# openjamoses/TOSEM-2021-Replication

Measured on NVIDIA H100. Metric: source MB/s scanned (tokenise + line-hash + classify + aggregate), higher is better.
Workload: dtype u8

## Files before the change

### tosem-2021-replication_b200/csrc/tsm_api.cu

```cuda
#include <algorithm>
#include <cstdio>
#include <cstdlib>
#include <cstring>
#include <new>
#include <vector>

#include "tsm_device.cuh"

#include "tsm_scan_kernels.cuh"
#include "tsm_scan_walk.cuh"
#include "tsm_reduce_kernels.cuh"
#include "tsm_diff_kernels.cuh"
#include "tsm_stmt_kernels.cuh"
#include "tsm_lines_kernels.cuh"

using namespace tsm;

static const char* const kNames[TSM_K] = TSM_CAT_NAMES_INIT;

struct ScratchPool {
  struct Slot { void* p; size_t cap; bool used; };
  std::vector<Slot> slots;
  void* take(size_t bytes) {
    int best = -1;
// ... 379 lines not shown
        }
      }
      p.slab = c->d_slab + s; p.f_begin = f0; p.f_end = f1;
      p.unit_base = (uint32_t)((host ? (int64_t)host->off[f0] : 0) / CH + f0);
      k_plan<<<(f1 - f0 + 255) / 256, 256, 0, st>>>(p);
      CU(cudaGetLastError());
      if (s == 0 && n_slabs == 1) CU(cudaEventRecord(ev[1], st));
      if (flags & TSM_SCAN_REV_B) k_scan_t<true><<<c->sms * SCAN2_CTAS_PER_SM, SCAN2_WARPS * 32, SCAN2_SMEM_B, st>>>(p);
      else k_scan_t<false><<<c->sms * SCAN2_CTAS_PER_SM, SCAN2_WARPS * 32, SCAN2_SMEM, st>>>(p);
      CU(cudaGetLastError());
      if (s + 1 < n_slabs) {
        p.cls_last = 0;
        if (flags & TSM_SCAN_REV_B) k_classify_t<true><<<c->cls_grid, 256, hist, st>>>(p);
        else k_classify_t<false><<<c->cls_grid, 256, hist, st>>>(p);
        CU(cudaGetLastError());
        p.cls_last = 1;
      }
    }
    if (n_slabs > 1) CU(cudaEventRecord(ev[1], st));
    CU(cudaEventRecord(ev[2], st));
    if (flags & TSM_SCAN_REV_B) k_classify_t<true><<<c->cls_grid, 256, hist, st>>>(p);
    else k_classify_t<false><<<c->cls_grid, 256, hist, st>>>(p);
    CU(cudaGetLastError());
    CU(cudaEventRecord(ev[3], st));
    CU(cudaEventRecord(ev[4], st));
    c->ev_used[es] = (n_slabs == 1);
    c->ev_last = es;
    c->launches = 3 * n_slabs;
    CU(cudaGetLastError());
  }
  c->last_flags = flags;
  c->scanned = true;
  return TSM_OK;
}

extern "C" int tsm_scan_resident(tsm_ctx* c, uint32_t flags, void* stream) {
  if (!c) return TSM_E_ARG;
  flags &= TSM_SCAN_ASSERT_EVENTS | TSM_SCAN_HEADER_EVENTS | TSM_SCAN_REV_B;
  if (!c->resident) return TSM_E_STATE;
  CU(cudaSetDevice(c->device));
  return launch_scan(c, flags, (cudaStream_t)stream, nullptr);
}

extern "C" int tsm_device_counts(tsm_ctx* c, void** dptr, int64_t* n_int64) {
  if (!c || !dptr || !n_int64) return TSM_E_ARG;
  if (!c->scanned) return TSM_E_STATE;
  *dptr = c->d_counts;
  *n_int64 = (int64_t)(c->n_groups + 1) * TSM_K + 4;
  return TSM_OK;
}

extern "C" int tsm_last_launch_count(tsm_ctx* c) { return c ? c->launches : 0; }

extern "C" int tsm_last_kernel_ms(tsm_ctx* c, float* ms4) {
  if (!c || !ms4) return TSM_E_ARG;
  if (!c->scanned || c->n_files == 0 || c->ev_last < 0) return TSM_E_STATE;
  CU(cudaSetDevice(c->device));
  cudaEvent_t* ev = c->ev[c->ev_last];
  CU(cudaEventSynchronize(ev[4]));
  for (int i = 0; i < 4; ++i) CU(cudaEventElapsedTime(&ms4[i], ev[i], ev[i + 1]));
  return TSM_OK;
}

extern "C" int tsm_kernel_ms_stats(tsm_ctx* c, double* sum_ms4, int64_t* n_scans, int reset) {
  if (!c) return TSM_E_ARG;
  CU(cudaSetDevice(c->device));
  for (int i = 0; i < tsm_ctx::kRing; ++i) fold_events(c, i);
  if (sum_ms4) for (int k = 0; k < 4; ++k) sum_ms4[k] = c->ms_sum[k];
  if (n_scans) *n_scans = c->ms_n;
  if (reset) { for (double& v : c->ms_sum) v = 0; c->ms_n = 0; }
  return TSM_OK;
}

extern "C" int tsm_download(tsm_ctx* c, tsm_result* r, void* stream) {
  if (!c || !r) return TSM_E_ARG;
  if (!c->scanned) return TSM_E_STATE;
  CU(cudaSetDevice(c->device));
  cudaStream_t st = (cudaStream_t)stream;
  const int n = c->n_files, G = c->n_groups;
  unsigned long long* h_tot = reinterpret_cast<unsigned long long*>(c->h_ctrl + 1);
  CU(cudaMemcpyAsync(c->h_ctrl, c->d_ctrl, sizeof(Ctrl), cudaMemcpyDeviceToHost, st));
  CU(cudaMemcpyAsync(h_tot, c->d_counts + (size_t)(G + 1) * TSM_K, 4 * sizeof(unsigned long long), cudaMemcpyDeviceToHost, st));
  if (r->stats && n) CU(cudaMemcpyAsync(r->stats, c->d_stats, sizeof(tsm_file_stat) * (size_t)n, cudaMemcpyDeviceToHost, st));
  if (r->group_counts) CU(cudaMemcpyAsync(r->group_counts, c->d_counts, sizeof(int64_t) * (size_t)G * TSM_K, cudaMemcpyDeviceToHost, st));
  if (r->global_counts) CU(cudaMemcpyAsync(r->global_counts, c->d_counts + (size_t)G * TSM_K, sizeof(int64_t) * TSM_K, cudaMemcpyDeviceToHost, st));
  CU(cudaStreamSynchronize(st));
  for (int i = 0; i < 4; ++i) r->totals[i] = (int64_t)h_tot[i];
  r->n_aev = 0; r->n_hev = 0;
  if (c->h_ctrl->overflow) return TSM_E_CAPACITY;
  if ((c->last_flags & TSM_SCAN_ASSERT_EVENTS) && r->aev) {
    const int64_t m = c->h_ctrl->n_aev;
    if (m > r->aev_cap) { r->n_aev = m; return TSM_E_CAPACITY; }
    CU(cudaMemcpyAsync(r->aev, c->d_aev, sizeof(tsm_assert_event) * (size_t)m, cudaMemcpyDeviceToHost, st));
    CU(cudaStreamSynchronize(st));
    std::sort(r->aev, r->aev + m, [](const tsm_assert_event& a, const tsm_assert_event& b) {
      return a.file != b.file ? a.file < b.file : a.line_off < b.line_off; });
    r->n_aev = m;
  } else if (c->last_flags & TSM_SCAN_ASSERT_EVENTS) r->n_aev = c->h_ctrl->n_aev;
  if ((c->last_flags & TSM_SCAN_HEADER_EVENTS) && r->hev) {
    const int64_t m = c->h_ctrl->n_hev;
    if (m > r->hev_cap) { r->n_hev = m; return TSM_E_CAPACITY; }
    CU(cudaMemcpyAsync(r->hev, c->d_hev, sizeof(tsm_header_event) * (size_t)m, cudaMemcpyDeviceToHost, st));
    CU(cudaStreamSynchronize(st));
    std::sort(r->hev, r->hev + m, [](const tsm_header_event& a, const tsm_header_event& b) {
      return a.file != b.file ? a.file < b.file : a.line_off < b.line_off; });
    r->n_hev = m;
// ... 523 lines not shown
```

### tosem-2021-replication_b200/csrc/tsm_scan_kernels.cuh

```cuda
#pragma once
#include <type_traits>
#include "tsm_device.cuh"

namespace tsm {

__constant__ uint32_t c_lut[256];
__constant__ uint32_t c_lut_b[256];
__constant__ uint32_t c_elut[256];
__device__ uint8_t c_cat_slot[TSM_CAT_SLOTS];
__device__ uint16_t c_cat_off[TSM_CAT_NAMED + 1];
__device__ char c_cat_blob[TSM_CAT_BLOB_LEN + 1];

__global__ void k_plan(ScanParams p) {
  const int f = p.f_begin + blockIdx.x * blockDim.x + threadIdx.x;
  const int lane = threadIdx.x & 31;
  if (blockIdx.x == 0 && threadIdx.x == 0) p.ctrl->cls_done = p.ctrl->n_cand;
  uint32_t nu = 0;
  if (f < p.f_end) {
    nu = ((uint32_t)p.len[f] + CH - 1) / CH;
    if (nu != 1) p.stats[f] = tsm_file_stat{0, 0, 0, 0, 0};
  }
  uint32_t incl = nu;
#pragma unroll
  for (int d = 1; d < 32; d <<= 1) {
// ... 112 lines not shown
template <typename LoadByte>
__device__ __forceinline__ uint32_t line_finish_h(uint32_t s, uint32_t e, unsigned long long h0, uint32_t nib, int ext,
                                                  LoadByte lb, Accum& ac) {
  uint32_t len = e - s;
  unsigned long long h = 0;
  if (len) {
    h = h0;
    if (lb(e - 1) == 0x0D) {
      --len;
      const unsigned long long cr = rotl61(0x0Dull, (8u * len) % 61u);
      h = h >= cr ? h - cr : h + M61 - cr;
    }
  }
  ac.lines++;
  ac.digest += mix_hash(h, len);
  if (ext == 0) return 0;
  uint32_t fl = (nib & 1u) ? LF_CAND : 0;
  bool hdr;
  if (ext == TSM_EXT_PY) {
    hdr = (nib & 2u) != 0;
    if (!hdr && (nib & 4u)) hdr = starts_with(lb, s, e, "class", 5, true);
  } else {
    hdr = (nib & 6u) == 6u;
  }
  if (hdr) { fl |= LF_HDR; if (starts_with(lb, s, e, "TEST_F", 6, false)) fl |= LF_FIX; }
  ac.asserts += fl & LF_CAND;
  ac.hdrs += (fl >> 1) & 1u;
  ac.fixes += (fl >> 2) & 1u;
  return fl;
}

template <typename LoadByte>
__device__ __forceinline__ uint32_t line_finish(uint32_t s, uint32_t e, uint32_t A, unsigned long long B, int ext,
                                                LoadByte lb, Accum& ac) {
  unsigned long long h0 = 0;
  if (e != s) {
    const uint32_t lead = s & 7u, m = ((e - 1) >> 3) - (s >> 3) + 1;
    h0 = rotl61(canon61(B), (3u * (m - 1) + 61u * 8u - 8u * lead) % 61u);
  }
  return line_finish_h(s, e, h0, ext ? flag_nibble_ext(A, ext) : 0u, ext, lb, ac);
}

__device__ __forceinline__ uint32_t warp_reserve(uint32_t* counter, uint32_t n, int lane) {
  uint32_t base = 0;
  if (lane == 0 && n) base = atomicAdd(counter, n);
  return __shfl_sync(0xffffffffu, base, 0);
}

__device__ __forceinline__ const uint32_t* scan_lut() {
  extern __shared__ __align__(128) uint8_t smem[];
  return reinterpret_cast<const uint32_t*>(smem);
}

__device__ __noinline__ uint32_t long_line(const ScanParams& p, const uint32_t* lut, uint32_t first, uint32_t f,
                                           uint32_t fo, uint32_t size, int ext, uint32_t s, Accum& ac, uint32_t* fl_out = nullptr) {
  const uint8_t* g = p.arena + fo;
  const GmemByte lb{g};
  uint32_t e = s;
  while (e < size && lb(e) != '\n') ++e;
  LineState L;
  line_init(L, s, e);
  while (L.pos < L.e) {
    const unsigned long long w = __ldg(reinterpret_cast<const unsigned long long*>(g + L.pos));
    line_block(L, w, lut, first);
  }
  const uint32_t fl = line_finish(s, e, L.A, L.B, ext, lb, ac);
  if ((fl & LF_CAND) && p.cand_cap) {
    const uint32_t slot = atomicAdd(&p.ctrl->n_cand, 1u);
    if (slot < p.cand_cap) p.cand[slot] = ((unsigned long long)f << 32) | s;
    else p.ctrl->overflow = 1;
  }
  if ((fl & LF_HDR) && (p.flags & TSM_SCAN_HEADER_EVENTS)) {
    const uint32_t slot = atomicAdd(&p.ctrl->n_hev, 1u);
    if (slot < p.hev_cap) p.hev[slot] = tsm_header_event{f, s, e - s, (fl >> 2) & 1u};
    else p.ctrl->overflow = 1;
  }
  if (fl_out) *fl_out = fl;
  return e;
}

__device__ __forceinline__ void issue_load(const ScanParams& p, uint8_t* buf, uint64_t* bar, uint32_t fo,
                                           uint32_t size, uint32_t cb) {
  const uint32_t lb = cb ? cb - PRE : 0u;
  const uint32_t le = min(cb + CH + EXT, size);
  const uint32_t bytes = (le - lb + 15u) & ~15u;
  mbar_expect_tx(bar, bytes);
  bulk_load(buf + PRE - (cb - lb), p.arena + (size_t)fo + lb, bytes, bar);
}

struct Unit { uint32_t u, f, cb, fo, size; int ext; };

__device__ __forceinline__ Unit claim_unit(const ScanParams& p, uint32_t n_units, int lane) {
  Unit x{0, 0, 0, 0, 0, 0};
  if (lane == 0) x.u = atomicAdd(&p.slab->work, 1u);
  x.u = __shfl_sync(0xffffffffu, x.u, 0);
  if (x.u < n_units) {
    x.f = p.unit_file[p.unit_base + x.u];
    x.cb = p.unit_begin[p.unit_base + x.u];
    x.fo = (uint32_t)p.off[x.f];
    x.size = (uint32_t)p.len[x.f];
    x.ext = p.ext[x.f];
  }
  return x;
}

constexpr uint32_t CC_W = 1, CC_IDENT = 2, CC_STOP = 4;
constexpr uint32_t CLS_CAT_OFF_N = (TSM_CAT_NAMED + 2) & ~1u;
constexpr uint32_t CLS_CAT_WORDS = ((TSM_CAT_SLOTS + 2 * CLS_CAT_OFF_N + TSM_CAT_BLOB_LEN + 15) / 16) * 4;
constexpr uint32_t CLS_SMEM_BASE = 4 * (512 + CLS_CAT_WORDS + 4 * 1024 + 4);
constexpr uint32_t E_FIRST = (1u << 0) | (1u << 5) | (1u << 9) | (1u << 17) | (1u << 21) | (1u << 23) | (1u << 25) |
                             (1u << 27) | (1u << 29) | (1u << 30);

struct FileBytes {
  const unsigned long long* base; uint32_t cur_blk; unsigned long long w;
  uint32_t blk0; unsigned long long w0, w1, w2, w3;
  __device__ __forceinline__ FileBytes(const uint8_t* b, uint32_t first_byte)
      : base(reinterpret_cast<const unsigned long long*>(b)), cur_blk(0xFFFFFFFFu), w(0), blk0(first_byte >> 3) {
    w0 = __ldg(base + blk0); w1 = __ldg(base + blk0 + 1); w2 = __ldg(base + blk0 + 2); w3 = __ldg(base + blk0 + 3);
  }
  __device__ __forceinline__ unsigned long long word(uint32_t blk) const {
    const uint32_t d = blk - blk0;
    if (d < 4u) return d < 2u ? (d == 0u ? w0 : w1) : (d == 2u ? w2 : w3);
    return __ldg(base + blk);
  }
  __device__ __forceinline__ uint32_t get(uint32_t i) {
    const uint32_t blk = i >> 3;
    if (blk != cur_blk) { w = word(blk); cur_blk = blk; }
    return (uint32_t)(w >> (8u * (i & 7u))) & 0xFFu;
  }
  __device__ __forceinline__ unsigned long long get8(uint32_t i) const {
    const uint32_t blk = i >> 3, sh = 8u * (i & 7u);
// ... 271 lines not shown
```

### tosem-2021-replication_b200/csrc/tsm_scan_walk.cuh

```cuda
#pragma once
#include "tsm_scan_kernels.cuh"

namespace tsm {

#ifndef TSM_SCAN2_WARPS
#define TSM_SCAN2_WARPS 11
#endif
#ifndef TSM_SCAN2_CTAS
#define TSM_SCAN2_CTAS 2
#endif
#ifndef TSM_RW2_SHIFT
#define TSM_RW2_SHIFT 2
#endif
#ifndef TSM_WALK_UNROLL
#define TSM_WALK_UNROLL 1
#endif
constexpr int SCAN2_WARPS = TSM_SCAN2_WARPS, SCAN2_CTAS_PER_SM = TSM_SCAN2_CTAS, WALK_UNROLL = TSM_WALK_UNROLL;

constexpr uint32_t NWORD = BUF / 8;
constexpr uint32_t O2_ARUN = BUF;
constexpr uint32_t SLOT_TAIL = NWORD;
constexpr uint32_t RW2_SHIFT = TSM_RW2_SHIFT, RW2_PER_STRIPE = 16u >> RW2_SHIFT;
constexpr uint32_t O2_RW = O2_ARUN + ((NWORD + 1) * 4 + 7) / 8 * 8;
constexpr uint32_t O2_WENT = O2_RW + 32 * RW2_PER_STRIPE * 8;
constexpr uint32_t WENT_CAP = NWORD + 8;
constexpr uint32_t LCAP = 512;
constexpr uint32_t O2_LTAB = O2_WENT + WENT_CAP * 2;
constexpr uint32_t O2_BASE = O2_LTAB + (LCAP + 8) * 2;
constexpr uint32_t Q2_CAP = 64;
constexpr uint32_t O2_Q = O2_BASE + 34 * 8;
constexpr uint32_t O2_CTL = O2_Q + Q2_CAP * 2;
constexpr uint32_t WARP_SMEM2 = ((O2_CTL + 16 + 127) / 128) * 128;
constexpr uint32_t O2_T0A = LUT_BYTES;
constexpr uint32_t CTA_BYTES2 = LUT_BYTES + 512;
constexpr uint32_t SCAN2_SMEM = CTA_BYTES2 + SCAN2_WARPS * WARP_SMEM2;
constexpr uint32_t O2_LUTB = SCAN2_SMEM;
constexpr uint32_t SCAN2_SMEM_B = SCAN2_SMEM + 1024;
static_assert(O2_RW % 8 == 0 && O2_WENT % 8 == 0 && O2_LTAB % 2 == 0 && O2_BASE % 8 == 0 && O2_Q % 4 == 0 && O2_CTL % 8 == 0, "alignment");
static_assert(SCAN2_CTAS_PER_SM * (SCAN2_SMEM_B + 1024) <= 233472, "shared memory per SM (228 KB, 1 KB reserved per CTA)");
constexpr uint32_t LR_POS = 0x1FFFu, LR_FIRST = 0x2000u, LR_MIXED = 0x4000u, LR_VIRT = 0x8000u;

constexpr uint32_t B2_FIRST = (1u << 0) | (1u << 6) | (1u << 15), B2_FIN = (1u << 5) | (1u << 14) | (1u << 18);
constexpr uint32_t REVB_BIT = 1u;

#ifndef TSM_PIPE_BALANCE
#define TSM_PIPE_BALANCE 1
#endif
template <bool REVB>
__device__ __forceinline__ void lut_at(uint32_t idx, uint32_t four, uint32_t& v, uint32_t& v2) {
#if TSM_PIPE_BALANCE
  uint32_t addr;
  asm("mad.lo.u32 %0, %1, %2, %3;" : "=r"(addr) : "r"(idx), "r"(four), "r"(smem_u32(scan_lut())));
  asm("ld.shared.u32 %0, [%1];" : "=r"(v) : "r"(addr));
  if (REVB) asm("ld.shared.u32 %0, [%1+%2];" : "=r"(v2) : "r"(addr), "n"(O2_LUTB));
#else
  (void)four;
  v = scan_lut()[idx];
  if (REVB) v2 = scan_lut()[O2_LUTB / 4 + idx];
#endif
}
__device__ __forceinline__ uint32_t opaque_four() { return scan_lut()[256 + 12]; }

struct Auto { uint32_t D, D2; };

template <bool REVB>
__device__ __forceinline__ uint32_t step1(Auto& a, uint32_t byte, uint32_t four) {
  uint32_t m, m2 = 0;
  lut_at<REVB>(byte, four, m, m2);
  a.D = ((a.D + a.D) | B_FIRST) & m;
  if (!REVB) return a.D;
  a.D2 = ((a.D2 + a.D2) | B2_FIRST) & m2;
  return (a.D & ~REVB_BIT) | ((a.D2 & B2_FIN) ? REVB_BIT : 0u);
}

template <bool REVB>
__device__ __forceinline__ void step8b(unsigned long long w, Auto& a, uint32_t& A, uint32_t four) {
  const uint32_t lo = (uint32_t)w, hi = (uint32_t)(w >> 32);
  uint32_t A2 = 0;
#pragma unroll
  for (int k = 0; k < 8; ++k) {
    uint32_t m, m2 = 0;
    lut_at<REVB>(__byte_perm(k < 4 ? lo : hi, 0, 0x4440 + (k & 3)), four, m, m2);
    a.D = ((a.D + a.D) | B_FIRST) & m;
    A |= a.D;
    if (REVB) { a.D2 = ((a.D2 + a.D2) | B2_FIRST) & m2; A2 |= a.D2; }
  }
  if (REVB) A = (A & ~REVB_BIT) | ((A2 & B2_FIN) ? REVB_BIT : 0u);
}

__device__ __forceinline__ uint32_t nl8_of(unsigned long long w) {
  return nl_word((uint32_t)w) | (nl_word((uint32_t)(w >> 32)) << 4);
}
__device__ __forceinline__ unsigned long long low_mask(uint32_t b) {
  return b >= 8u ? ~0ull : ((1ull << (8u * b)) - 1ull);
}
__device__ __forceinline__ unsigned long long ror3_61(unsigned long long r) { return (r >> 3) + ((r & 7ull) << 58); }

struct WalkOut { uint32_t nlw, tail; };

template <bool REVB>
__device__ __noinline__ WalkOut walk2(uint8_t* wb, uint32_t fin, int lane) {
  const uint32_t pos0 = (uint32_t)lane * STRIPE;
  const uint8_t* sp = wb + pos0;
  uint32_t* ar = reinterpret_cast<uint32_t*>(wb + O2_ARUN) + (uint32_t)lane * 17u;
  unsigned long long* rw = reinterpret_cast<unsigned long long*>(wb + O2_RW) + (uint32_t)lane * RW2_PER_STRIPE;
  const uint32_t four = opaque_four();
  Auto au{0u, 0u};
  if (lane) {
    uint32_t A = 0;
    step8b<REVB>(*reinterpret_cast<const unsigned long long*>(sp - 8), au, A, four);
  }
  unsigned long long R = 0;
  uint32_t run = 0, nlr = 0;
#pragma unroll 1
  for (uint32_t g = 0; g < 5; ++g) {
#pragma unroll WALK_UNROLL
    for (uint32_t k = 0; k < 4; ++k) {
      if (g == 4 && k) break;
      const unsigned long long w = *reinterpret_cast<const unsigned long long*>(sp + 32u * g + 8u * k);
      uint32_t A = 0;
      step8b<REVB>(w, au, A, four);
      R = ror3_61(R) + fold61(w);
      if (((k + 1u) & ((1u << RW2_SHIFT) - 1u)) == 0u && g < 4u) rw[(4u * g + k) >> RW2_SHIFT] = R;
      ar[4u * g + k] = run;
      nlr = __funnelshift_l(A, nlr, 1);
      const bool nl = (int32_t)A < 0;
      if (nl && (A & fin)) {
        const uint32_t slot = atomicAdd(reinterpret_cast<uint32_t*>(wb + O2_CTL), 1u);
        if (slot < Q2_CAP) reinterpret_cast<uint16_t*>(wb + O2_Q)[slot] = (uint16_t)((uint32_t)lane * 17u + 4u * g + k);
      }
      run = nl ? 0u : (run | A);
    }
  }
  unsigned long long incl = rotl61(canon61(R), (3u * (17u * (uint32_t)lane + 16u)) % 61u);
#pragma unroll
  for (int d = 1; d < 32; d <<= 1) {
    const unsigned long long t = __shfl_up_sync(0xffffffffu, incl, d);
    if (lane >= d) incl = fold61(incl + t);
  }
  unsigned long long excl = __shfl_up_sync(0xffffffffu, incl, 1);
  if (lane == 0) excl = 0;
  unsigned long long* sbase = reinterpret_cast<unsigned long long*>(wb + O2_BASE);
  sbase[lane] = excl;
  if (lane == 31) sbase[32] = incl;
  return WalkOut{__brev(nlr) >> 15, run};
}

template <bool REVB>
__device__ __noinline__ void resolve_mixed(uint8_t* wb, uint32_t g, uint32_t i, uint32_t n_went) {
  const uint32_t four = opaque_four();
  Auto au{0u, 0u};
  uint32_t A = 0;
  step8b<REVB>(*reinterpret_cast<const unsigned long long*>(wb + 8u * g - 8u), au, A, four);
  unsigned long long w = *reinterpret_cast<const unsigned long long*>(wb + 8u * g);
  uint32_t pre = 0, post = 0, seen = 0;
#pragma unroll
  for (int b = 0; b < 8; ++b) {
    const uint32_t d = step1<REVB>(au, (uint32_t)w & 0xFFu, four);
    const uint32_t m = (uint32_t)((int32_t)au.D >> 31);
    pre |= d & ~seen;
    seen |= m;
    post = (post | d) & ~m;
    w >>= 8;
  }
  uint32_t* arun = reinterpret_cast<uint32_t*>(wb + O2_ARUN);
  const uint16_t* went = reinterpret_cast<const uint16_t*>(wb + O2_WENT);
  atomicOr(arun + g, pre);
  const uint32_t tgt = i + 1u < n_went ? ((uint32_t)went[i + 1u] & 0x3FFu) : SLOT_TAIL;
  atomicOr(arun + tgt, post);
}

__device__ __forceinline__ void emit_header(const ScanParams& p, uint32_t f, uint32_t line_off, uint32_t len, uint32_t fl) {
  const uint32_t slot = atomicAdd(&p.ctrl->n_hev, 1u);
  if (slot < p.hev_cap) p.hev[slot] = tsm_header_event{f, line_off, len, (fl >> 2) & 1u};
  else p.ctrl->overflow = 1;
}

__device__ __noinline__ bool starts_with8(SmemByte lb, uint32_t s, uint32_t e, unsigned long long pat, uint32_t n, bool need_ws) {
  uint32_t r;
  while (s + 8 <= e && (r = lb.spaces8(s)) != 0) { s += r; if (r < 8) break; }
  while (s < e && is_w(lb(s))) ++s;
  if (s + n + (need_ws ? 1u : 0u) > e) return false;
  const unsigned long long v = lb.load8(s);
  if ((v & low_mask(n)) != pat) return false;
  if (need_ws) {
    const uint32_t c = (uint32_t)(v >> (8u * n)) & 0xFFu;
    if (c != 0x20 && c != 0x09) return false;
    for (uint32_t q = s + n + 1; q < e; ++q)
      if (!is_w(lb(q))) return true;
    return false;
  }
  return true;
}

template <bool REVB>
__device__ __forceinline__ uint32_t line_flags2(uint32_t s, uint32_t e, uint32_t A, uint32_t g1, uint32_t g2, int ext, SmemByte lb, Accum& ac) {
  if (ext == 0) return 0;
  uint32_t fl = (A & (AF_ASSERT | AF_EXPECT | (REVB ? REVB_BIT : 0u))) ? LF_CAND : 0;
  bool hdr;
  if (ext == TSM_EXT_PY) {
    hdr = (A & g1) != 0;
    if (!hdr && (A & g2)) hdr = starts_with8(lb, s, e, 0x7373616C63ull, 5, true);
  } else {
    hdr = (A & g1) != 0 && (A & g2) != 0;
  }
  if (hdr) { fl |= LF_HDR; if ((A & B_F) && starts_with8(lb, s, e, 0x465F54534554ull, 6, false)) fl |= LF_FIX; }
  ac.asserts += fl & LF_CAND;
  ac.hdrs += (fl >> 1) & 1u;
  ac.fixes += (fl >> 2) & 1u;
  return fl;
}

__device__ __noinline__ bool revb_trigger_gmem(const uint8_t* g, uint32_t s, uint32_t e) {
  const char* const pats[3] = {"_CHECK", "TESTEQUAL", "FAIL"};
  const uint32_t lens[3] = {6, 9, 4};
  for (int t = 0; t < 3; ++t)
    for (uint32_t i = s; i + lens[t] <= e; ++i) {
      uint32_t k = 0;
      while (k < lens[t] && __ldg(g + i + k) == (uint8_t)pats[t][k]) ++k;
      if (k == lens[t]) return true;
    }
  return false;
}

struct FinishState {
  uint32_t prev_last;
  unsigned long long prevP;
  uint32_t lh_base, lh_done;
};

template <bool REVB>
__device__ __noinline__ void finish_lines2(const ScanParams& p, uint8_t* wb, const uint32_t* lc, uint32_t n, uint32_t lim,
                                           bool skip_first, uint32_t f, uint32_t cb, int ext, int lane, Accum& ac, FinishState& fs) {
  uint16_t* ltab = reinterpret_cast<uint16_t*>(wb + O2_LTAB);
  const uint32_t* arun = reinterpret_cast<const uint32_t*>(wb + O2_ARUN);
  const unsigned long long* t0a = reinterpret_cast<const unsigned long long*>(scan_lut()) + O2_T0A / 8;
  const uint32_t g1 = lc[1], g2 = lc[2];
  const SmemByte lb{wb};
  const bool want_hev = (p.flags & TSM_SCAN_HEADER_EVENTS) != 0, want_lh = (p.flags & TSM_SCAN_LINE_HASHES) != 0;
  Accum a = ac;
  uint32_t nc = 0, lh_done = fs.lh_done;
  uint32_t prev_last = fs.prev_last;
  unsigned long long prevP = fs.prevP;
  for (uint32_t base = 0; base < n; base += 32) {
    const uint32_t j = base + (uint32_t)lane;
    const bool valid = j < n;
    const uint32_t rec = valid ? (uint32_t)ltab[j] : 0u;
    const uint32_t e = rec & LR_POS;
    const bool isv = (rec & LR_VIRT) != 0;
    const uint32_t g = min(e >> 3, NWORD - 1u), b1 = e - 8u * g + (isv ? 0u : 1u);
    const uint32_t l = g / 17u, i = g - 17u * l, c0 = i >> RW2_SHIFT, ns = i & ((1u << RW2_SHIFT) - 1u);
    unsigned long long R = 0;
    if (c0) R = *reinterpret_cast<const unsigned long long*>(wb + O2_RW + 8u * (l * RW2_PER_STRIPE + c0 - 1u));
    const unsigned long long* wp = reinterpret_cast<const unsigned long long*>(wb) + (g - ns);
#pragma unroll
    for (uint32_t t = 0; t + 1u < (1u << RW2_SHIFT); ++t)
      if (ns > t) R = ror3_61(R) + fold61(wp[t]);
    const unsigned long long w = *reinterpret_cast<const unsigned long long*>(wb + 8u * g);
    const uint32_t r3g = (3u * g) % 61u;
    const unsigned long long X = ror3_61(R) + fold61(w & low_mask(b1));
    unsigned long long Pn = *reinterpret_cast<const unsigned long long*>(wb + O2_BASE + 8u * l) + rotl61(fold61(fold61(X)), r3g);
    uint32_t r8e = r3g + 8u * (e & 7u);
    if (r8e >= 61u) r8e -= 61u;
    const unsigned long long Pe = isv ? Pn : Pn + M61 - t0a[r8e];
    uint32_t s = __shfl_up_sync(0xffffffffu, e, 1) + 1u;
    unsigned long long Ps = __shfl_up_sync(0xffffffffu, Pn, 1);
    if (lane == 0) { s = prev_last + 1u; Ps = prevP; }
    const int src = base + 32u <= n ? 31 : (int)(n - 1u - base);
    prev_last = __shfl_sync(0xffffffffu, e, src);
    prevP = __shfl_sync(0xffffffffu, Pn, src);
    const bool owned = valid && s < lim && !(s == PRE && skip_first);
    uint32_t fl = 0;
    unsigned long long lh = 0;
    if (owned) {
      const unsigned long long hr = canon61(Pe + 4ull * M61 - Ps);
      const uint32_t sh = (8u * s) % 61u;
      unsigned long long h = rotl61(hr, sh ? 61u - sh : 0u);
      uint32_t len = e - s;
      if (len && lb(e - 1u) == 0x0D) {
        --len;
        const unsigned long long cr = rotl61(0x0Dull, (8u * len) % 61u);
        h = h >= cr ? h - cr : h + M61 - cr;
      }
      a.lines++;
      lh = mix_hash(h, len);
      a.digest += lh;
      uint32_t A = 0;
      if (rec & LR_FIRST) A = arun[isv ? SLOT_TAIL : g];
      else if (rec & LR_MIXED) {
        Auto au{0u, 0u};
        const uint32_t four = opaque_four();
        for (uint32_t q = s; q < e; ++q) A |= step1<REVB>(au, lb(q), four);
      }
      fl = line_flags2<REVB>(s, e, A, g1, g2, ext, lb, a);
      if (want_hev && (fl & LF_HDR)) emit_header(p, f, cb + s - PRE, e - s, fl);
    }
    if (want_lh) {
      const uint32_t mo = __ballot_sync(0xffffffffu, owned);
      const uint32_t slot = fs.lh_base + lh_done + __popc(mo & ((1u << lane) - 1u));
      if (owned && slot < p.lh_cap) {
        p.lh_hash[slot] = lh;
        p.lh_end[slot] = cb + e - PRE;
        p.lh_flag[slot] = (uint8_t)(fl & LF_CAND);
      }
      lh_done += __popc(mo);
    }
    __syncwarp();
    const uint32_t mc = __ballot_sync(0xffffffffu, fl & LF_CAND);
    if (fl & LF_CAND) ltab[nc + __popc(mc & ((1u << lane) - 1u))] = (uint16_t)s;
    nc += __popc(mc);
  }
  __syncwarp();
  if (nc && p.cand_cap) {
    const uint32_t cbase = warp_reserve(&p.ctrl->n_cand, nc, lane);
    for (uint32_t i = (uint32_t)lane; i < nc; i += 32) {
      const uint32_t slot = cbase + i;
      if (slot < p.cand_cap) p.cand[slot] = ((unsigned long long)f << 32) | (cb + (uint32_t)ltab[i] - PRE);
      else p.ctrl->overflow = 1;
    }
  }
  __syncwarp();
  ac = a;
  fs.prev_last = prev_last;
  fs.prevP = prevP;
  fs.lh_done = lh_done;
}

template <bool REVB>
__device__ __forceinline__ void process_chunk2(const ScanParams& p, const uint32_t* lc, uint8_t* wb, uint32_t uslot, uint32_t f,
                                               uint32_t cb, uint32_t fo, uint32_t size, int ext, int lane) {
  const uint32_t ce = min(cb + CH, size);
  const uint32_t le = min(ce + EXT, size);
  const uint32_t lim = PRE + (ce - cb);
  const uint32_t lim2 = PRE + (le - cb);
  const bool skip_first = (cb != 0) && (wb[PRE - 1] != '\n');
  Accum ac{0, 0, 0, 0, 0};
  __syncwarp();
  if (lane < 2) reinterpret_cast<unsigned long long*>(wb)[lane] = 0ull;
  {
    const uint32_t za = (lim2 + 7u) & ~7u;
    if ((uint32_t)lane < za - lim2) wb[lim2 + lane] = 0;
    for (uint32_t q = za + 8u * (uint32_t)lane; q < BUF; q += 256u) *reinterpret_cast<unsigned long long*>(wb + q) = 0ull;
  }
  if (lane == 0) *reinterpret_cast<uint32_t*>(wb + O2_CTL) = 0u;
  __syncwarp();
  const WalkOut wo = walk2<REVB>(wb, lc[0], lane);
  const uint32_t w0 = 17u * (uint32_t)lane, lim_w = (lim + 7u) >> 3;
  const uint32_t ownbits = lim_w <= w0 ? 0u : (lim_w - w0 >= 17u ? 0x1FFFFu : (1u << (lim_w - w0)) - 1u);
  const uint32_t extbits = wo.nlw & ~ownbits;
  const uint32_t gx = __reduce_min_sync(0xffffffffu, extbits ? w0 + (uint32_t)__ffs((int)extbits) - 1u : 0xFFFFu);
  uint32_t kept = wo.nlw & ownbits;
  if (gx - w0 < 17u) kept |= 1u << (gx - w0);
  uint32_t tv = wo.tail, tf = wo.nlw != 0u;
  const uint32_t cnt = __popc(kept);
  uint32_t incl = cnt;
#pragma unroll
  for (int d = 1; d < 32; d <<= 1) {
    const uint32_t uv = __shfl_up_sync(0xffffffffu, tv, d), uf = __shfl_up_sync(0xffffffffu, tf, d);
    const uint32_t t = __shfl_up_sync(0xffffffffu, incl, d);
    if (lane >= d) { if (!tf) tv |= uv; tf |= uf; incl += t; }
  }
  uint32_t carry = __shfl_up_sync(0xffffffffu, tv, 1);
  if (lane == 0) carry = 0;
  const uint32_t tail_all = __shfl_sync(0xffffffffu, tv, 31);
  const uint32_t n_went = __shfl_sync(0xffffffffu, incl, 31), ebase = incl - cnt;
  uint16_t* went = reinterpret_cast<uint16_t*>(wb + O2_WENT);
  uint32_t* arun = reinterpret_cast<uint32_t*>(wb + O2_ARUN);
  {
    uint32_t b = kept, idx = ebase;
    while (b) { went[idx++] = (uint16_t)(w0 + (uint32_t)__ffs((int)b) - 1u); b &= b - 1u; }
    if (wo.nlw) arun[w0 + (uint32_t)__ffs((int)wo.nlw) - 1u] |= carry;
    if (lane == 0) arun[SLOT_TAIL] = tail_all;
  }
  __syncwarp();
  {
    const uint32_t nq_all = *reinterpret_cast<const uint32_t*>(wb + O2_CTL);
    const uint16_t* q = reinterpret_cast<const uint16_t*>(wb + O2_Q);
    if (nq_all <= Q2_CAP) {
      for (uint32_t base = 0; base < nq_all; base += 32) {
        const uint32_t t = base + (uint32_t)lane;
        const uint32_t g = t < nq_all ? (uint32_t)q[t] : 0u;
        const uint32_t l = g / 17u, k = g - 17u * l;
        const uint32_t m = __shfl_sync(0xffffffffu, kept, (int)l), eb = __shfl_sync(0xffffffffu, ebase, (int)l);
        const bool act = t < nq_all && ((m >> k) & 1u);
        const uint32_t i = eb + __popc(m & ((1u << k) - 1u));
        if (act) resolve_mixed<REVB>(wb, g, i, n_went);
        __syncwarp();
        if (act) went[i] |= 0x8000u;
        __syncwarp();
      }
    } else if (lc[0]) {
      for (uint32_t base = 0; base < n_went; base += 32) {
        const uint32_t i = base + (uint32_t)lane;
        if (i < n_went) resolve_mixed<REVB>(wb, (uint32_t)went[i] & 0x3FFu, i, n_went);
        __syncwarp();
        if (i < n_went) went[i] |= 0x8000u;
        __syncwarp();
      }
    }
  }
  uint16_t* ltab = reinterpret_cast<uint16_t*>(wb + O2_LTAB);
  FinishState fs{PRE - 1u, 0ull, 0u, 0u};
  const bool want_lh = (p.flags & TSM_SCAN_LINE_HASHES) != 0;
  if (want_lh) {
    uint32_t tot = 0;
    for (uint32_t j = (uint32_t)lane; j < n_went; j += 32)
      tot += __popc(nl8_of(*reinterpret_cast<const unsigned long long*>(wb + 8u * ((uint32_t)went[j] & 0x3FFu))));
    tot = __reduce_add_sync(0xffffffffu, tot) + 1u;
    uint32_t base = 0;
    if (lane == 0) {
      base = atomicAdd(&p.ctrl->n_lh, tot);
      if (base + tot > p.lh_cap) p.ctrl->lh_overflow = 1;
      p.unit_out[uslot] = base;
    }
    fs.lh_base = __shfl_sync(0xffffffffu, base, 0);
  }
  uint32_t n_rec = 0, last_nl = PRE - 1u;
  for (uint32_t base = 0; base < n_went; base += 32) {
    const uint32_t j = base + (uint32_t)lane;
    const uint32_t ge = j < n_went ? (uint32_t)went[j] : 0u;
    const uint32_t g = ge & 0x3FFu;
    uint32_t m = j < n_went ? nl8_of(*reinterpret_cast<const unsigned long long*>(wb + 8u * g)) : 0u;
    const uint32_t c = __popc(m);
    uint32_t in2 = c;
#pragma unroll
    for (int d = 1; d < 32; d <<= 1) {
      const uint32_t t = __shfl_up_sync(0xffffffffu, in2, d);
      if (lane >= d) in2 += t;
    }
    if (base + 32u >= n_went) {
      const uint32_t lastl = n_went - 1u - base;
      last_nl = __shfl_sync(0xffffffffu, 8u * g + 31u - (uint32_t)__clz((int)(m | 1u)), (int)lastl);
    }
    uint32_t off = n_rec + in2 - c;
    uint32_t rec = 8u * g + LR_FIRST + ((ge >> 15) << 14);
    while (m) {
      ltab[off++] = (uint16_t)(rec + (uint32_t)__ffs((int)m) - 1u);
      rec &= ~LR_FIRST;
      m &= m - 1u;
    }
    n_rec += __shfl_sync(0xffffffffu, in2, 31);
    __syncwarp();
    if (n_rec + 256u > LCAP && base + 32u < n_went) {
      finish_lines2<REVB>(p, wb, lc, n_rec, lim, skip_first, f, cb, ext, lane, ac, fs);
      n_rec = 0;
    }
  }
  const uint32_t tail_start = last_nl + 1u;
  bool tail_long = false;
  if (tail_start < lim && !(skip_first && n_went == 0u)) {
    if (le == size) {
      if (tail_start < lim2) { if (lane == 0) ltab[n_rec] = (uint16_t)(lim2 | LR_VIRT | LR_FIRST); ++n_rec; }
    } else tail_long = true;
  }
  __syncwarp();
  if (n_rec) finish_lines2<REVB>(p, wb, lc, n_rec, lim, skip_first, f, cb, ext, lane, ac, fs);
  if (tail_long && lane == 0) {
    const unsigned long long d0 = ac.digest;
    uint32_t fl = 0;
    const uint32_t ls = cb + tail_start - PRE;
    const uint32_t e = long_line(p, scan_lut(), B_FIRST, f, fo, size, ext, ls, ac, &fl);
    if (REVB && ext != 0 && !(fl & LF_CAND) && revb_trigger_gmem(p.arena + fo, ls, e)) {
      fl |= LF_CAND;
      ac.asserts++;
      if (p.cand_cap) {
        const uint32_t slot = atomicAdd(&p.ctrl->n_cand, 1u);
        if (slot < p.cand_cap) p.cand[slot] = ((unsigned long long)f << 32) | ls;
        else p.ctrl->overflow = 1;
      }
    }
    if (want_lh) {
      const uint32_t slot = fs.lh_base + fs.lh_done;
      if (slot < p.lh_cap) { p.lh_hash[slot] = ac.digest - d0; p.lh_end[slot] = e; p.lh_flag[slot] = (uint8_t)(fl & LF_CAND); }
    }
  }
  ac.lines = __reduce_add_sync(0xffffffffu, ac.lines);
  ac.asserts = __reduce_add_sync(0xffffffffu, ac.asserts);
  ac.hdrs = __reduce_add_sync(0xffffffffu, ac.hdrs);
  ac.fixes = __reduce_add_sync(0xffffffffu, ac.fixes);
  {
    const uint32_t dlo = (uint32_t)ac.digest, dhi = (uint32_t)(ac.digest >> 32);
    const unsigned long long s0 = __reduce_add_sync(0xffffffffu, dlo & 0xFFFFu);
    const unsigned long long s1 = __reduce_add_sync(0xffffffffu, dlo >> 16);
    const unsigned long long s2 = __reduce_add_sync(0xffffffffu, dhi);
    ac.digest = s0 + (s1 << 16) + (s2 << 32);
  }
  if (want_lh && lane == 0) p.unit_lines[uslot] = ac.lines;
  if (lane == 0) {
    tsm_file_stat* st = p.stats + f;
    if (size <= CH) {
      *st = tsm_file_stat{ac.lines, ac.asserts, ac.hdrs, ac.fixes, ac.digest};
    } else {
      if (ac.lines) atomicAdd(&st->n_lines, ac.lines);
      if (ac.asserts) atomicAdd(&st->n_assert, ac.asserts);
      if (ac.hdrs) atomicAdd(&st->n_headers, ac.hdrs);
      if (ac.fixes) atomicAdd(&st->n_fixture, ac.fixes);
      if (ac.digest) atomicAdd(reinterpret_cast<unsigned long long*>(&st->digest), ac.digest);
    }
  }
}

template <bool REVB>
__global__ void __launch_bounds__(SCAN2_WARPS * 32, SCAN2_CTAS_PER_SM) k_scan_t(ScanParams p) {
  extern __shared__ __align__(128) uint8_t smem[];
  uint32_t* lut_all = reinterpret_cast<uint32_t*>(smem);
  for (int i = threadIdx.x; i < 256; i += blockDim.x) lut_all[i] = c_lut[i];
  if (threadIdx.x < 12) {
    const int t = threadIdx.x, lang = t >> 2, q = t & 3;
    const uint32_t g1 = lang == 0 ? PY_G1 : CJ_G1, g2 = lang == 0 ? PY_G2 : CJ_G2;
    const uint32_t v = q == 0 ? (AF_ASSERT | AF_EXPECT | g1 | g2 | B_F | (REVB ? REVB_BIT : 0u)) : (q == 1 ? g1 : (q == 2 ? g2 : 0u));
    lut_all[256 + t] = lang == 2 ? 0u : v;
  }
  if (threadIdx.x == 12) lut_all[256 + 12] = p.four;
  if (REVB) for (int i = threadIdx.x; i < 256; i += blockDim.x) lut_all[O2_LUTB / 4 + i] = c_lut_b[i];
  if (threadIdx.x >= 32 && threadIdx.x < 32 + 61)
    reinterpret_cast<unsigned long long*>(smem + O2_T0A)[threadIdx.x - 32] = rotl61(0x0Aull, threadIdx.x - 32);
  __syncthreads();
  const int warp = threadIdx.x >> 5, lane = threadIdx.x & 31;
  uint8_t* wb = smem + CTA_BYTES2 + warp * WARP_SMEM2;
  uint64_t* bar = reinterpret_cast<uint64_t*>(wb + O2_CTL + 8);
  if (lane == 0) { mbar_init(bar, 1); fence_mbar_init(); }
  __syncwarp();
  const uint32_t n_units = p.slab->n_units;
  uint32_t phase = 0;
  Unit cur = claim_unit(p, n_units, lane);
#ifndef TSM_LOCKSTEP2
#define TSM_LOCKSTEP2 0
#endif
#if TSM_LOCKSTEP2
  while (__syncthreads_or(cur.u < n_units)) {
    if (cur.u >= n_units) continue;
#else
  while (cur.u < n_units) {
#endif
    fence_proxy_async();
    __syncwarp();
    if (lane == 0) issue_load(p, wb, bar, cur.fo, cur.size, cur.cb);
    const Unit nxt = claim_unit(p, n_units, lane);
    while (!mbar_try_wait(bar, phase)) {}
    phase ^= 1;
    const uint32_t lang = cur.ext == 0 ? 2u : (cur.ext == TSM_EXT_PY ? 0u : 1u);
    process_chunk2<REVB>(p, lut_all + 256u + 4u * lang, wb, p.unit_base + cur.u, cur.f, cur.cb, cur.fo, cur.size, cur.ext, lane);
    __syncwarp();
    cur = nxt;
  }
}

template __global__ void k_scan_t<false>(ScanParams);
template __global__ void k_scan_t<true>(ScanParams);

}
```

Baseline: 551,400.

## Cut scan-kernel register pressure and add optional per-phase clock profiling

Adds compile-time-gated per-phase clock64 instrumentation for the scan kernel, off by default. Also reduces live registers: the LUT base address and the `four` value are cached in shared memory, the mbarrier phase moves to shared memory, `fo` is reloaded from p.off instead of being carried, and noinline helpers return their state by value instead of through reference parameters. The walk loop is restructured with a fixed stripe of 4 words and a peeled 17th word, and the kernel parameter is marked __grid_constant__. The extra shared-memory loads and stores could add latency.

```diff
diff --git a/tosem-2021-replication_b200/csrc/tsm_api.cu b/tosem-2021-replication_b200/csrc/tsm_api.cu
--- a/tosem-2021-replication_b200/csrc/tsm_api.cu
+++ b/tosem-2021-replication_b200/csrc/tsm_api.cu
@@ -455,6 +455,19 @@
 
 extern "C" int tsm_last_launch_count(tsm_ctx* c) { return c ? c->launches : 0; }
 
+#if TSM_PHASE_CLOCKS
+extern "C" int tsm_phase_clocks(unsigned long long* out, int n, int reset) {
+  if (!out || n < (int)PH_N) return TSM_E_ARG;
+  CU(cudaDeviceSynchronize());
+  CU(cudaMemcpyFromSymbol(out, g_scan_phase_clk, sizeof(unsigned long long) * PH_N));
+  if (reset) {
+    const unsigned long long zero[PH_N] = {};
+    CU(cudaMemcpyToSymbol(g_scan_phase_clk, zero, sizeof(zero)));
+  }
+  return TSM_OK;
+}
+#endif
+
 extern "C" int tsm_last_kernel_ms(tsm_ctx* c, float* ms4) {
   if (!c || !ms4) return TSM_E_ARG;
   if (!c->scanned || c->n_files == 0 || c->ev_last < 0) return TSM_E_STATE;
diff --git a/tosem-2021-replication_b200/csrc/tsm_scan_kernels.cuh b/tosem-2021-replication_b200/csrc/tsm_scan_kernels.cuh
--- a/tosem-2021-replication_b200/csrc/tsm_scan_kernels.cuh
+++ b/tosem-2021-replication_b200/csrc/tsm_scan_kernels.cuh
@@ -188,8 +188,9 @@
   return reinterpret_cast<const uint32_t*>(smem);
 }
 
-__device__ __noinline__ uint32_t long_line(const ScanParams& p, const uint32_t* lut, uint32_t first, uint32_t f,
-                                           uint32_t fo, uint32_t size, int ext, uint32_t s, Accum& ac, uint32_t* fl_out = nullptr) {
+struct LongLine { uint32_t e, fl; Accum ac; };
+__device__ __noinline__ LongLine long_line(const ScanParams& p, const uint32_t* lut, uint32_t first, uint32_t f,
+                                           uint32_t fo, uint32_t size, int ext, uint32_t s, Accum ac) {
   const uint8_t* g = p.arena + fo;
   const GmemByte lb{g};
   uint32_t e = s;
@@ -211,8 +212,7 @@
     if (slot < p.hev_cap) p.hev[slot] = tsm_header_event{f, s, e - s, (fl >> 2) & 1u};
     else p.ctrl->overflow = 1;
   }
-  if (fl_out) *fl_out = fl;
-  return e;
+  return LongLine{e, fl, ac};
 }
 
 __device__ __forceinline__ void issue_load(const ScanParams& p, uint8_t* buf, uint64_t* bar, uint32_t fo,
diff --git a/tosem-2021-replication_b200/csrc/tsm_scan_walk.cuh b/tosem-2021-replication_b200/csrc/tsm_scan_walk.cuh
--- a/tosem-2021-replication_b200/csrc/tsm_scan_walk.cuh
+++ b/tosem-2021-replication_b200/csrc/tsm_scan_walk.cuh
@@ -8,9 +8,6 @@
 #endif
 #ifndef TSM_SCAN2_CTAS
 #define TSM_SCAN2_CTAS 2
-#endif
-#ifndef TSM_RW2_SHIFT
-#define TSM_RW2_SHIFT 2
 #endif
 #ifndef TSM_WALK_UNROLL
 #define TSM_WALK_UNROLL 1
@@ -20,7 +17,7 @@
 constexpr uint32_t NWORD = BUF / 8;
 constexpr uint32_t O2_ARUN = BUF;
 constexpr uint32_t SLOT_TAIL = NWORD;
-constexpr uint32_t RW2_SHIFT = TSM_RW2_SHIFT, RW2_PER_STRIPE = 16u >> RW2_SHIFT;
+constexpr uint32_t RW2_PER_STRIPE = 4;
 constexpr uint32_t O2_RW = O2_ARUN + ((NWORD + 1) * 4 + 7) / 8 * 8;
 constexpr uint32_t O2_WENT = O2_RW + 32 * RW2_PER_STRIPE * 8;
 constexpr uint32_t WENT_CAP = NWORD + 8;
@@ -31,8 +28,30 @@
 constexpr uint32_t O2_Q = O2_BASE + 34 * 8;
 constexpr uint32_t O2_CTL = O2_Q + Q2_CAP * 2;
 constexpr uint32_t WARP_SMEM2 = ((O2_CTL + 16 + 127) / 128) * 128;
+#ifndef TSM_PHASE_CLOCKS
+#define TSM_PHASE_CLOCKS 0
+#endif
+enum ScanPhase { PH_WAIT, PH_ZERO, PH_WALK, PH_SCANS, PH_MIXED, PH_RECORDS, PH_FINISH, PH_LONG, PH_FLUSH, PH_N };
+#if TSM_PHASE_CLOCKS
+__device__ unsigned long long g_scan_phase_clk[PH_N];
+#endif
+struct PhaseClock {
+#if TSM_PHASE_CLOCKS
+  uint32_t* tab;
+  long long t;
+  __device__ __forceinline__ void mark(int ph, int lane) {
+    const long long now = clock64();
+    if (lane == 0) atomicAdd(tab + ph, (uint32_t)(now - t));
+    t = now;
+  }
+#else
+  __device__ __forceinline__ void mark(int, int) {}
+#endif
+};
+
 constexpr uint32_t O2_T0A = LUT_BYTES;
-constexpr uint32_t CTA_BYTES2 = LUT_BYTES + 512;
+constexpr uint32_t O2_PHASE = LUT_BYTES + 512;
+constexpr uint32_t CTA_BYTES2 = LUT_BYTES + 512 + (TSM_PHASE_CLOCKS ? 128 : 0);
 constexpr uint32_t SCAN2_SMEM = CTA_BYTES2 + SCAN2_WARPS * WARP_SMEM2;
 constexpr uint32_t O2_LUTB = SCAN2_SMEM;
 constexpr uint32_t SCAN2_SMEM_B = SCAN2_SMEM + 1024;
@@ -46,27 +65,28 @@
 #ifndef TSM_PIPE_BALANCE
 #define TSM_PIPE_BALANCE 1
 #endif
-template <bool REVB>
-__device__ __forceinline__ void lut_at(uint32_t idx, uint32_t four, uint32_t& v, uint32_t& v2) {
+struct LutRef { uint32_t four, base; };
+__device__ __forceinline__ LutRef lut_ref() { return LutRef{scan_lut()[256 + 12], scan_lut()[256 + 13]}; }
+template <bool REVB>
+__device__ __forceinline__ void lut_at(uint32_t idx, LutRef t, uint32_t& v, uint32_t& v2) {
 #if TSM_PIPE_BALANCE
   uint32_t addr;
-  asm("mad.lo.u32 %0, %1, %2, %3;" : "=r"(addr) : "r"(idx), "r"(four), "r"(smem_u32(scan_lut())));
+  asm("mad.lo.u32 %0, %1, %2, %3;" : "=r"(addr) : "r"(idx), "r"(t.four), "r"(t.base));
   asm("ld.shared.u32 %0, [%1];" : "=r"(v) : "r"(addr));
   if (REVB) asm("ld.shared.u32 %0, [%1+%2];" : "=r"(v2) : "r"(addr), "n"(O2_LUTB));
 #else
-  (void)four;
+  (void)t;
   v = scan_lut()[idx];
   if (REVB) v2 = scan_lut()[O2_LUTB / 4 + idx];
 #endif
 }
-__device__ __forceinline__ uint32_t opaque_four() { return scan_lut()[256 + 12]; }
 
 struct Auto { uint32_t D, D2; };
 
 template <bool REVB>
-__device__ __forceinline__ uint32_t step1(Auto& a, uint32_t byte, uint32_t four) {
+__device__ __forceinline__ uint32_t step1(Auto& a, uint32_t byte, LutRef t) {
   uint32_t m, m2 = 0;
-  lut_at<REVB>(byte, four, m, m2);
+  lut_at<REVB>(byte, t, m, m2);
   a.D = ((a.D + a.D) | B_FIRST) & m;
   if (!REVB) return a.D;
   a.D2 = ((a.D2 + a.D2) | B2_FIRST) & m2;
@@ -74,13 +94,13 @@
 }
 
 template <bool REVB>
-__device__ __forceinline__ void step8b(unsigned long long w, Auto& a, uint32_t& A, uint32_t four) {
+__device__ __forceinline__ void step8b(unsigned long long w, Auto& a, uint32_t& A, LutRef t) {
   const uint32_t lo = (uint32_t)w, hi = (uint32_t)(w >> 32);
   uint32_t A2 = 0;
 #pragma unroll
   for (int k = 0; k < 8; ++k) {
     uint32_t m, m2 = 0;
-    lut_at<REVB>(__byte_perm(k < 4 ? lo : hi, 0, 0x4440 + (k & 3)), four, m, m2);
+    lut_at<REVB>(__byte_perm(k < 4 ? lo : hi, 0, 0x4440 + (k & 3)), t, m, m2);
     a.D = ((a.D + a.D) | B_FIRST) & m;
     A |= a.D;
     if (REVB) { a.D2 = ((a.D2 + a.D2) | B2_FIRST) & m2; A2 |= a.D2; }
@@ -104,34 +124,35 @@
   const uint8_t* sp = wb + pos0;
   uint32_t* ar = reinterpret_cast<uint32_t*>(wb + O2_ARUN) + (uint32_t)lane * 17u;
   unsigned long long* rw = reinterpret_cast<unsigned long long*>(wb + O2_RW) + (uint32_t)lane * RW2_PER_STRIPE;
-  const uint32_t four = opaque_four();
+  const LutRef t = lut_ref();
   Auto au{0u, 0u};
   if (lane) {
     uint32_t A = 0;
-    step8b<REVB>(*reinterpret_cast<const unsigned long long*>(sp - 8), au, A, four);
+    step8b<REVB>(*reinterpret_cast<const unsigned long long*>(sp - 8), au, A, t);
   }
   unsigned long long R = 0;
   uint32_t run = 0, nlr = 0;
+  auto word = [&](uint32_t k) {
+    const unsigned long long w = *reinterpret_cast<const unsigned long long*>(sp + 8u * k);
+    uint32_t A = 0;
+    step8b<REVB>(w, au, A, t);
+    R = ror3_61(R) + fold61(w);
+    ar[k] = run;
+    nlr = __funnelshift_l(A, nlr, 1);
+    const bool nl = (int32_t)A < 0;
+    if (nl && (A & fin)) {
+      const uint32_t slot = atomicAdd(reinterpret_cast<uint32_t*>(wb + O2_CTL), 1u);
+      if (slot < Q2_CAP) reinterpret_cast<uint16_t*>(wb + O2_Q)[slot] = (uint16_t)((uint32_t)lane * 17u + k);
+    }
+    run = nl ? 0u : (run | A);
+  };
 #pragma unroll 1
-  for (uint32_t g = 0; g < 5; ++g) {
+  for (uint32_t g = 0; g < 4; ++g) {
 #pragma unroll WALK_UNROLL
-    for (uint32_t k = 0; k < 4; ++k) {
-      if (g == 4 && k) break;
-      const unsigned long long w = *reinterpret_cast<const unsigned long long*>(sp + 32u * g + 8u * k);
-      uint32_t A = 0;
-      step8b<REVB>(w, au, A, four);
-      R = ror3_61(R) + fold61(w);
-      if (((k + 1u) & ((1u << RW2_SHIFT) - 1u)) == 0u && g < 4u) rw[(4u * g + k) >> RW2_SHIFT] = R;
-      ar[4u * g + k] = run;
-      nlr = __funnelshift_l(A, nlr, 1);
-      const bool nl = (int32_t)A < 0;
-      if (nl && (A & fin)) {
-        const uint32_t slot = atomicAdd(reinterpret_cast<uint32_t*>(wb + O2_CTL), 1u);
-        if (slot < Q2_CAP) reinterpret_cast<uint16_t*>(wb + O2_Q)[slot] = (uint16_t)((uint32_t)lane * 17u + 4u * g + k);
-      }
-      run = nl ? 0u : (run | A);
-    }
-  }
+    for (uint32_t k = 0; k < 4; ++k) word(4u * g + k);
+    rw[g] = R;
+  }
+  word(16);
   unsigned long long incl = rotl61(canon61(R), (3u * (17u * (uint32_t)lane + 16u)) % 61u);
 #pragma unroll
   for (int d = 1; d < 32; d <<= 1) {
@@ -148,15 +169,15 @@
 
 template <bool REVB>
 __device__ __noinline__ void resolve_mixed(uint8_t* wb, uint32_t g, uint32_t i, uint32_t n_went) {
-  const uint32_t four = opaque_four();
+  const LutRef t = lut_ref();
   Auto au{0u, 0u};
   uint32_t A = 0;
-  step8b<REVB>(*reinterpret_cast<const unsigned long long*>(wb + 8u * g - 8u), au, A, four);
+  step8b<REVB>(*reinterpret_cast<const unsigned long long*>(wb + 8u * g - 8u), au, A, t);
   unsigned long long w = *reinterpret_cast<const unsigned long long*>(wb + 8u * g);
   uint32_t pre = 0, post = 0, seen = 0;
 #pragma unroll
   for (int b = 0; b < 8; ++b) {
-    const uint32_t d = step1<REVB>(au, (uint32_t)w & 0xFFu, four);
+    const uint32_t d = step1<REVB>(au, (uint32_t)w & 0xFFu, t);
     const uint32_t m = (uint32_t)((int32_t)au.D >> 31);
     pre |= d & ~seen;
     seen |= m;
@@ -224,21 +245,22 @@
 }
 
 struct FinishState {
+  Accum ac;
   uint32_t prev_last;
   unsigned long long prevP;
   uint32_t lh_base, lh_done;
 };
 
 template <bool REVB>
-__device__ __noinline__ void finish_lines2(const ScanParams& p, uint8_t* wb, const uint32_t* lc, uint32_t n, uint32_t lim,
-                                           bool skip_first, uint32_t f, uint32_t cb, int ext, int lane, Accum& ac, FinishState& fs) {
+__device__ __noinline__ FinishState finish_lines2(const ScanParams& p, uint8_t* wb, const uint32_t* lc, uint32_t n, uint32_t lim,
+                                                  bool skip_first, uint32_t f, uint32_t cb, int ext, int lane, FinishState fs) {
   uint16_t* ltab = reinterpret_cast<uint16_t*>(wb + O2_LTAB);
   const uint32_t* arun = reinterpret_cast<const uint32_t*>(wb + O2_ARUN);
   const unsigned long long* t0a = reinterpret_cast<const unsigned long long*>(scan_lut()) + O2_T0A / 8;
   const uint32_t g1 = lc[1], g2 = lc[2];
   const SmemByte lb{wb};
   const bool want_hev = (p.flags & TSM_SCAN_HEADER_EVENTS) != 0, want_lh = (p.flags & TSM_SCAN_LINE_HASHES) != 0;
-  Accum a = ac;
+  Accum a = fs.ac;
   uint32_t nc = 0, lh_done = fs.lh_done;
   uint32_t prev_last = fs.prev_last;
   unsigned long long prevP = fs.prevP;
@@ -249,12 +271,12 @@
     const uint32_t e = rec & LR_POS;
     const bool isv = (rec & LR_VIRT) != 0;
     const uint32_t g = min(e >> 3, NWORD - 1u), b1 = e - 8u * g + (isv ? 0u : 1u);
-    const uint32_t l = g / 17u, i = g - 17u * l, c0 = i >> RW2_SHIFT, ns = i & ((1u << RW2_SHIFT) - 1u);
+    const uint32_t l = g / 17u, i = g - 17u * l, c0 = i >> 2, ns = i & 3u;
     unsigned long long R = 0;
     if (c0) R = *reinterpret_cast<const unsigned long long*>(wb + O2_RW + 8u * (l * RW2_PER_STRIPE + c0 - 1u));
     const unsigned long long* wp = reinterpret_cast<const unsigned long long*>(wb) + (g - ns);
 #pragma unroll
-    for (uint32_t t = 0; t + 1u < (1u << RW2_SHIFT); ++t)
+    for (uint32_t t = 0; t < 3u; ++t)
       if (ns > t) R = ror3_61(R) + fold61(wp[t]);
     const unsigned long long w = *reinterpret_cast<const unsigned long long*>(wb + 8u * g);
     const uint32_t r3g = (3u * g) % 61u;
@@ -289,8 +311,8 @@
       if (rec & LR_FIRST) A = arun[isv ? SLOT_TAIL : g];
       else if (rec & LR_MIXED) {
         Auto au{0u, 0u};
-        const uint32_t four = opaque_four();
-        for (uint32_t q = s; q < e; ++q) A |= step1<REVB>(au, lb(q), four);
+        const LutRef t = lut_ref();
+        for (uint32_t q = s; q < e; ++q) A |= step1<REVB>(au, lb(q), t);
       }
       fl = line_flags2<REVB>(s, e, A, g1, g2, ext, lb, a);
       if (want_hev && (fl & LF_HDR)) emit_header(p, f, cb + s - PRE, e - s, fl);
@@ -320,21 +342,21 @@
     }
   }
   __syncwarp();
-  ac = a;
+  fs.ac = a;
   fs.prev_last = prev_last;
   fs.prevP = prevP;
   fs.lh_done = lh_done;
+  return fs;
 }
 
 template <bool REVB>
 __device__ __forceinline__ void process_chunk2(const ScanParams& p, const uint32_t* lc, uint8_t* wb, uint32_t uslot, uint32_t f,
-                                               uint32_t cb, uint32_t fo, uint32_t size, int ext, int lane) {
+                                               uint32_t cb, uint32_t size, int ext, int lane, PhaseClock& pc) {
   const uint32_t ce = min(cb + CH, size);
   const uint32_t le = min(ce + EXT, size);
   const uint32_t lim = PRE + (ce - cb);
   const uint32_t lim2 = PRE + (le - cb);
   const bool skip_first = (cb != 0) && (wb[PRE - 1] != '\n');
-  Accum ac{0, 0, 0, 0, 0};
   __syncwarp();
   if (lane < 2) reinterpret_cast<unsigned long long*>(wb)[lane] = 0ull;
   {
@@ -344,7 +366,9 @@
   }
   if (lane == 0) *reinterpret_cast<uint32_t*>(wb + O2_CTL) = 0u;
   __syncwarp();
+  pc.mark(PH_ZERO, lane);
   const WalkOut wo = walk2<REVB>(wb, lc[0], lane);
+  pc.mark(PH_WALK, lane);
   const uint32_t w0 = 17u * (uint32_t)lane, lim_w = (lim + 7u) >> 3;
   const uint32_t ownbits = lim_w <= w0 ? 0u : (lim_w - w0 >= 17u ? 0x1FFFFu : (1u << (lim_w - w0)) - 1u);
   const uint32_t extbits = wo.nlw & ~ownbits;
@@ -373,6 +397,7 @@
     if (lane == 0) arun[SLOT_TAIL] = tail_all;
   }
   __syncwarp();
+  pc.mark(PH_SCANS, lane);
   {
     const uint32_t nq_all = *reinterpret_cast<const uint32_t*>(wb + O2_CTL);
     const uint16_t* q = reinterpret_cast<const uint16_t*>(wb + O2_Q);
@@ -399,8 +424,9 @@
       }
     }
   }
+  pc.mark(PH_MIXED, lane);
   uint16_t* ltab = reinterpret_cast<uint16_t*>(wb + O2_LTAB);
-  FinishState fs{PRE - 1u, 0ull, 0u, 0u};
+  FinishState fs{{0, 0, 0, 0, 0}, PRE - 1u, 0ull, 0u, 0u};
   const bool want_lh = (p.flags & TSM_SCAN_LINE_HASHES) != 0;
   if (want_lh) {
     uint32_t tot = 0;
@@ -442,7 +468,9 @@
     n_rec += __shfl_sync(0xffffffffu, in2, 31);
     __syncwarp();
     if (n_rec + 256u > LCAP && base + 32u < n_went) {
-      finish_lines2<REVB>(p, wb, lc, n_rec, lim, skip_first, f, cb, ext, lane, ac, fs);
+      pc.mark(PH_RECORDS, lane);
+      fs = finish_lines2<REVB>(p, wb, lc, n_rec, lim, skip_first, f, cb, ext, lane, fs);
+      pc.mark(PH_FINISH, lane);
       n_rec = 0;
     }
   }
@@ -454,12 +482,18 @@
     } else tail_long = true;
   }
   __syncwarp();
-  if (n_rec) finish_lines2<REVB>(p, wb, lc, n_rec, lim, skip_first, f, cb, ext, lane, ac, fs);
+  pc.mark(PH_RECORDS, lane);
+  if (n_rec) fs = finish_lines2<REVB>(p, wb, lc, n_rec, lim, skip_first, f, cb, ext, lane, fs);
+  pc.mark(PH_FINISH, lane);
+  Accum ac = fs.ac;
   if (tail_long && lane == 0) {
     const unsigned long long d0 = ac.digest;
-    uint32_t fl = 0;
     const uint32_t ls = cb + tail_start - PRE;
-    const uint32_t e = long_line(p, scan_lut(), B_FIRST, f, fo, size, ext, ls, ac, &fl);
+    const uint32_t fo = (uint32_t)p.off[f];
+    const LongLine ll = long_line(p, scan_lut(), B_FIRST, f, fo, size, ext, ls, ac);
+    const uint32_t e = ll.e;
+    uint32_t fl = ll.fl;
+    ac = ll.ac;
     if (REVB && ext != 0 && !(fl & LF_CAND) && revb_trigger_gmem(p.arena + fo, ls, e)) {
       fl |= LF_CAND;
       ac.asserts++;
@@ -474,6 +508,7 @@
       if (slot < p.lh_cap) { p.lh_hash[slot] = ac.digest - d0; p.lh_end[slot] = e; p.lh_flag[slot] = (uint8_t)(fl & LF_CAND); }
     }
   }
+  pc.mark(PH_LONG, lane);
   ac.lines = __reduce_add_sync(0xffffffffu, ac.lines);
   ac.asserts = __reduce_add_sync(0xffffffffu, ac.asserts);
   ac.hdrs = __reduce_add_sync(0xffffffffu, ac.hdrs);
@@ -498,10 +533,11 @@
       if (ac.digest) atomicAdd(reinterpret_cast<unsigned long long*>(&st->digest), ac.digest);
     }
   }
-}
-
-template <bool REVB>
-__global__ void __launch_bounds__(SCAN2_WARPS * 32, SCAN2_CTAS_PER_SM) k_scan_t(ScanParams p) {
+  pc.mark(PH_FLUSH, lane);
+}
+
+template <bool REVB>
+__global__ void __launch_bounds__(SCAN2_WARPS * 32, SCAN2_CTAS_PER_SM) k_scan_t(const __grid_constant__ ScanParams p) {
   extern __shared__ __align__(128) uint8_t smem[];
   uint32_t* lut_all = reinterpret_cast<uint32_t*>(smem);
   for (int i = threadIdx.x; i < 256; i += blockDim.x) lut_all[i] = c_lut[i];
@@ -512,18 +548,27 @@
     lut_all[256 + t] = lang == 2 ? 0u : v;
   }
   if (threadIdx.x == 12) lut_all[256 + 12] = p.four;
+  if (threadIdx.x == 13) lut_all[256 + 13] = smem_u32(lut_all);
   if (REVB) for (int i = threadIdx.x; i < 256; i += blockDim.x) lut_all[O2_LUTB / 4 + i] = c_lut_b[i];
+  PhaseClock pc;
+#if TSM_PHASE_CLOCKS
+  pc.tab = reinterpret_cast<uint32_t*>(smem + O2_PHASE);
+  if (threadIdx.x < PH_N) pc.tab[threadIdx.x] = 0u;
+#endif
   if (threadIdx.x >= 32 && threadIdx.x < 32 + 61)
     reinterpret_cast<unsigned long long*>(smem + O2_T0A)[threadIdx.x - 32] = rotl61(0x0Aull, threadIdx.x - 32);
   __syncthreads();
   const int warp = threadIdx.x >> 5, lane = threadIdx.x & 31;
   uint8_t* wb = smem + CTA_BYTES2 + warp * WARP_SMEM2;
   uint64_t* bar = reinterpret_cast<uint64_t*>(wb + O2_CTL + 8);
-  if (lane == 0) { mbar_init(bar, 1); fence_mbar_init(); }
+  uint32_t* phase = reinterpret_cast<uint32_t*>(wb + O2_CTL + 4);
+  if (lane == 0) { mbar_init(bar, 1); fence_mbar_init(); *phase = 0u; }
   __syncwarp();
   const uint32_t n_units = p.slab->n_units;
-  uint32_t phase = 0;
   Unit cur = claim_unit(p, n_units, lane);
+#if TSM_PHASE_CLOCKS
+  pc.t = clock64();
+#endif
 #ifndef TSM_LOCKSTEP2
 #define TSM_LOCKSTEP2 0
 #endif
@@ -537,16 +582,23 @@
     __syncwarp();
     if (lane == 0) issue_load(p, wb, bar, cur.fo, cur.size, cur.cb);
     const Unit nxt = claim_unit(p, n_units, lane);
-    while (!mbar_try_wait(bar, phase)) {}
-    phase ^= 1;
+    const uint32_t ph = *phase;
+    while (!mbar_try_wait(bar, ph)) {}
+    __syncwarp();
+    if (lane == 0) *phase = ph ^ 1u;
+    pc.mark(PH_WAIT, lane);
     const uint32_t lang = cur.ext == 0 ? 2u : (cur.ext == TSM_EXT_PY ? 0u : 1u);
-    process_chunk2<REVB>(p, lut_all + 256u + 4u * lang, wb, p.unit_base + cur.u, cur.f, cur.cb, cur.fo, cur.size, cur.ext, lane);
+    process_chunk2<REVB>(p, lut_all + 256u + 4u * lang, wb, p.unit_base + cur.u, cur.f, cur.cb, cur.size, cur.ext, lane, pc);
     __syncwarp();
     cur = nxt;
   }
-}
-
-template __global__ void k_scan_t<false>(ScanParams);
-template __global__ void k_scan_t<true>(ScanParams);
-
-}
+#if TSM_PHASE_CLOCKS
+  __syncthreads();
+  if (threadIdx.x < PH_N) atomicAdd(&g_scan_phase_clk[threadIdx.x], (unsigned long long)pc.tab[threadIdx.x]);
+#endif
+}
+
+template __global__ void k_scan_t<false>(const __grid_constant__ ScanParams);
+template __global__ void k_scan_t<true>(const __grid_constant__ ScanParams);
+
+}
```

Measured after the change: 599,800 (median of 6 runs). 8.8% higher.
